# wanxinjin/Learning-from-Sparse-Demonstrations

Hardware: NVIDIA B200
Metric: CPDP OCP gradient-iterations per second (batched quadrotor OCPs, n_grid 50) (higher is better)
Workload: dtype f64

## Files before the change

learning-from-sparse-demonstrations_b200/csrc/cpdp_bdf.cuh:

```cuda
#pragma once
#include "cpdp_aux.cuh"

namespace CPDP_NS {

constexpr int BDF_THREADS = 32;
constexpr int NC = NX + NP;
static_assert(NC <= 32, "k_riccati_bdf maps one lane per column of [P | W]");
static_assert(NX <= 15 && NP <= 16, "warp sections map one lane per row/column and 16 + lane for the second half / the rows of Z; lane 31 must stay free for the bulge-chase fix-up");
#ifndef CPDP_BDF_MINB
#define CPDP_BDF_MINB 8
#endif
constexpr int BDF_MAX_ORDER = 5;
constexpr int BDF_NEWTON_MAXITER = 4;
constexpr int BDF_NROWS = BDF_MAX_ORDER + 3;
constexpr int BDF_WS_DOUBLES = BDF_NROWS * NX * NC;

#ifndef CPDP_BDF_LMUL_UNROLL
#define CPDP_BDF_LMUL_UNROLL 1
#endif
#ifndef CPDP_BDF_STENCIL_UNROLL
#define CPDP_BDF_STENCIL_UNROLL 1
#endif
#ifdef __CUDACC__
#define BDF_SYNC() __syncwarp()
#define BDF_UNROLL _Pragma("unroll")
#define BDF_PRAGMA_STR(x) _Pragma(#x)
#define BDF_PRAGMA_UNROLL(n) BDF_PRAGMA_STR(unroll n)
#else
#define BDF_SYNC() __syncthreads()
#define BDF_UNROLL
#define BDF_PRAGMA_UNROLL(n)
#endif

CPDP_HD double bdf_kappa(int k) { const double v[6] = {0.0, -0.1850, -1.0 / 9, -0.0823, -0.0415, 0.0}; return v[k]; }
CPDP_HD double bdf_gamma(int k) { const double v[6] = {0.0, 1.0, 1.5, 1.8333333333333333, 2.083333333333333, 2.283333333333333}; return v[k]; }
CPDP_HD double bdf_alpha(int k) { return (1.0 - bdf_kappa(k)) * bdf_gamma(k); }
CPDP_HD double bdf_error_const(int k) { return bdf_kappa(k) * bdf_gamma(k) + 1.0 / (k + 1); }

#ifdef __CUDACC__
CPDP_D double bdf_mul(double a, double b) { return __dmul_rn(a, b); }
#else
CPDP_D double bdf_mul(double a, double b) { volatile double r = a * b; return r; }
#endif

constexpr int QS = (NX + 1) & ~1;
constexpr int NCS = NC | 1;
constexpr int SWQ = (NX - 1 + 3) / 4;
constexpr int TW = 4 * SWQ;
constexpr int NH = (NX + 1) / 2;
namespace bo {
constexpr int M = 0;
constexpr int XUL = M + ((MSZ + 1) & ~1);
constexpr int RED = XUL + ((2 * NX + NU + 1) & ~1);
constexpr int Q = RED + 66;
constexpr int QT = Q + NX * QS;
constexpr int WT = QT + NX * QS;
constexpr int LM = WT + NX * QS;
constexpr int Y2 = LM + ((NX * NX + 1) & ~1);
constexpr int T2S = Y2 + 2 * NX * NX;
constexpr int TD = T2S + 2 * NX * TW;
constexpr int PV = TD + 2 * NX;
constexpr int CM = PV + 2 * NX * NX;
constexpr int XA = CM + ((NX * NP + 1) & ~1);
constexpr int XB = XA + NX * NCS;
constexpr int GHM = XB + NX * NCS;
constexpr int YPM = GHM + NX * NU;
constexpr int ROT = YPM + NU * NX;
constexpr int RU = (ROT + 4 * NX + 1) & ~1;
constexpr int FLAG = RU + 128;
constexpr int NODE = FLAG + 2;
constexpr int NODE_W = 2 * NX + NU;
#ifdef CPDP_BDF_TIMING
constexpr int TS = NODE + ((2 * NODE_W + 1) & ~1);
constexpr int END = TS + 8;
#else
constexpr int END = NODE + ((2 * NODE_W + 1) & ~1);
#endif
static_assert(Y2 % 2 == 0 && T2S % 2 == 0 && TD % 2 == 0 && PV % 2 == 0 && RU % 2 == 0, "complex arrays are read with 128-bit loads");
}
constexpr int BDF_SMEM_DOUBLES = bo::END;
constexpr size_t BDF_SMEM_BYTES = (size_t)BDF_SMEM_DOUBLES * sizeof(double);

struct cplx { double x, y; };
#ifdef __CUDACC__
#define BDF_LD2(p) (*reinterpret_cast<const double2*>(p))
#define BDF_ST2(p, a, b) (*reinterpret_cast<double2*>(p) = make_double2((a), (b)))
#else
#define BDF_LD2(p) (*reinterpret_cast<const cplx*>(p))
#define BDF_ST2(p, a, b) do { (p)[0] = (a); (p)[1] = (b); } while (0)
#endif

#define BDF_SM() CPDP_DYN_SMEM(sm)

CPDP_D_NOINLINE double bdf_reduce(double v, bool is_max) {
#ifdef __CUDACC__
    BDF_UNROLL for (int o = 16; o > 0; o >>= 1) {
        const double x = __shfl_xor_sync(0xffffffffu, v, o);
        v = is_max ? fmax(v, x) : (v + x);
    }
    return v;
#else
    BDF_SM();
    return block_reduce(v, sm + bo::RED, is_max);
#endif
}
CPDP_D_NOINLINE double bdf_pow(double x, double y) { return pow(x, y); }
CPDP_D double bdf_rcp(double x) {
#ifdef __CUDACC__
    double r;
    asm("rcp.approx.ftz.f64 %0, %1;" : "=d"(r) : "d"(x));
    r = fma(r, fma(-x, r, 1.0), r);
    r = fma(r, fma(-x, r, 1.0), r);
    return r;
#else
    return 1.0 / x;
#endif
}

#ifdef CPDP_BDF_TIMING
#define BDF_T(ph, ...) do { const long long t0__ = clock64(); __VA_ARGS__; tp[ph] += clock64() - t0__; } while (0)
#define BDF_TB(ph, var, expr) do { const long long t0__ = clock64(); var = (expr); tp[ph] += clock64() - t0__; } while (0)
#define BDF_TP_PARAM , long long* tp
#define BDF_TP_ARG , tp
#define BDF_TS0() const long long ts0__ = clock64()
#define BDF_TS(i) do { if (threadIdx.x == 0) sm[bo::TS + (i)] += (double)(clock64() - ts0__); } while (0)
#else
#define BDF_T(ph, ...) do { __VA_ARGS__; } while (0)
#define BDF_TB(ph, var, expr) do { var = (expr); } while (0)
#define BDF_TP_PARAM
#define BDF_TP_ARG
#define BDF_TS0()
#define BDF_TS(i)
#endif

template <int AS>
CPDP_D_NOINLINE void bdf_lmul_t(const double* __restrict__ AT, const double* __restrict__ x, const int xs,
                                double* __restrict__ dst, const int ds, const int i0) {
    double out[NH];
    BDF_UNROLL for (int i = 0; i < NH; ++i) out[i] = 0.0;
    const double* A0 = AT + i0;
    BDF_PRAGMA_UNROLL(CPDP_BDF_LMUL_UNROLL) for (int k = 0; k < NX; ++k) {
        const double xk = x[k * xs];
        if constexpr (AS % 2 == 0 && (NX - NH) % 2 == 0) {
            double a[NH + 1];
            BDF_UNROLL for (int i = 0; i + 1 < NH + 1; i += 2) { const auto v = BDF_LD2(A0 + k * AS + i); a[i] = v.x; a[i + 1] = v.y; }
            BDF_UNROLL for (int i = 0; i < NH; ++i) out[i] += a[i] * xk;
        } else {
            BDF_UNROLL for (int i = 0; i < NH; ++i) out[i] += A0[k * AS + i] * xk;
        }
    }
    const int first = (i0 > 0) ? 2 * NH - NX : 0;
    BDF_UNROLL for (int i = 0; i < NH; ++i) if (i >= first) dst[(i0 + i) * ds] = out[i];
}
CPDP_D void bdf_lmul_to(const double* AT, const int as, const double* x, const int xs, double* dst, const int ds, const int i0) {
    if (as == QS) bdf_lmul_t<QS>(AT, x, xs, dst, ds, i0);
    else bdf_lmul_t<NCS>(AT, x, xs, dst, ds, i0);
}
CPDP_D bool bdf_half(const int lane, int& col, int& i0) {
    col = lane & 15;
    i0 = (lane >> 4) ? NX - NH : 0;
    return col < NX;
}
CPDP_D void bdf_put(double* buf, int c, const double (&v)[NX]) {
    BDF_UNROLL for (int i = 0; i < NX; ++i) buf[i * NCS + c] = v[i];
}
CPDP_D void bdf_get_col(const double* buf, int c, double (&v)[NX]) {
    BDF_UNROLL for (int i = 0; i < NX; ++i) v[i] = buf[i * NCS + c];
}

CPDP_D void bdf_stage_nodes(double* sm, const AuxProblem& p, const double t0) {
    const int lane = threadIdx.x;
    const int lo = interp_lo(t0, p.dt, p.N);
    BDF_SYNC();
    CPDP_LOOP for (int q = lane; q < 2 * bo::NODE_W; q += BDF_THREADS) {
        const int row = lo + q / bo::NODE_W, e = q % bo::NODE_W;
        sm[bo::NODE + q] = (e < NX) ? p.X[(size_t)row * NX + e]
                         : (e < NX + NU) ? p.U[(size_t)row * NU + e - NX] : p.Lam[(size_t)row * NX + e - NX - NU];
    }
    if (lane == 0) ((int*)(sm + bo::FLAG))[2] = lo;
    BDF_SYNC();
}
CPDP_D_NOINLINE bool bdf_prepare(const AuxProblem p, const double t) {
    BDF_SM();
    const int lane = threadIdx.x;
    BDF_SYNC();
// ... 288 lines not shown
                        pass = (u <= EPS * v);
                    }
                }
                m = bdf_top_bit(bdf_ballot(sm, pass));
                p = bdf_bcast(sm, p, m); q = bdf_bcast(sm, q, m); r = bdf_bcast(sm, r, m);
            }
            BDF_SYNC();
            if (lane == 0 && l >= 1) h_(l, l - 1) = 0.0;
            BDF_TS(1);
            CPDP_LOOP for (int k = m; k <= en - 1; ++k) {
                const bool notlast = (k != en - 1);
                SS(g_ss.steps++);
                if (k != m) { p = h_(k, k - 1); q = h_(k + 1, k - 1); r = notlast ? h_(k + 2, k - 1) : 0.0; }
                const double sig = p * p + q * q + r * r;
                if (sig == 0.0) continue;
                const double rs = bdf_rsqrt(sig);
                const double sgn = (p < 0.0) ? -1.0 : 1.0;
                const double s = sgn * (sig * rs);
                const double xx = 1.0 + fabs(p) * rs, yy = q * rs * sgn, zz = r * rs * sgn;
                const double ixx = bdf_rcp(xx);
                const double qn = yy * ixx, rn = zz * ixx;
                {
                    const bool on = lane >= k && lane < n;
                    double* const col = on ? H + lane : Z;
                    const double a0 = col[k * n], a1 = col[(k + 1) * n], a2 = notlast ? col[(k + 2) * n] : 0.0;
                    const double pp = (a0 + qn * a1) + rn * a2;
                    if (on && notlast) col[(k + 2) * n] = a2 - pp * zz;
                    if (on) col[k * n] = a0 - pp * xx;
                    if (on) col[(k + 1) * n] = a1 - pp * yy;
                }
                BDF_SYNC();
                {
                    const int imax = (en < k + 3) ? en : k + 3;
                    const bool on = lane < 16 ? (rw <= imax) : (rw < n);
                    const double z0 = Mrow[k], z1 = Mrow[k + 1], z2 = notlast ? Mrow[k + 2] : 0.0;
                    const double pp = (xx * z0 + yy * z1) + zz * z2;
                    if (on && notlast) Mrow[k + 2] = z2 - pp * rn;
                    if (on) Mrow[k] = z0 - pp;
                    if (on) Mrow[k + 1] = z1 - pp * qn;
                    if (lane == 31) {
                        if (k != m) { h_(k, k - 1) = -s; h_(k + 1, k - 1) = 0.0; if (notlast) h_(k + 2, k - 1) = 0.0; }
                        else if (l != m) h_(k, k - 1) = -h_(k, k - 1);
                    }
                }
                BDF_SYNC();
            }
            BDF_TS(2);
        }
    }
#undef h_
    return true;
}

CPDP_D_NOINLINE bool bdf_schur() {
    BDF_SM();
    constexpr int n = NX;
    const int lane = threadIdx.x;
    double* Tr = sm + bo::PV; double* Ti = Tr + n * n;
    double* Zm = sm + bo::Y2;
    double* ga = sm + bo::ROT; double* gbr = ga + n; double* gbi = gbr + n; double* pi = gbi + n;
    int* flag = (int*)(sm + bo::FLAG);
    BDF_SYNC();
    CPDP_LOOP for (int e = lane; e < n * n; e += BDF_THREADS) { Tr[e] = sm[bo::LM + e]; Ti[e] = 0.0; }
    if (lane == 0) flag[1] = 1;
    BDF_SYNC();
    const bool ok = schur_real_w0(sm, Tr, Zm, sm + bo::RU);
    BDF_SYNC();
    BDF_TS0();
    if (!ok && lane == 0) flag[1] = 0;
    if (lane < n) { ga[lane] = 1.0; gbr[lane] = 0.0; gbi[lane] = 0.0; pi[lane] = (double)lane; }
    BDF_SYNC();
    CPDP_LOOP for (int j = 0; ok && j < n - 1; ++j) {
        const double cc = Tr[(j + 1) * n + j];
        if (cc == 0.0) continue;
        const double a = Tr[j * n + j], b = Tr[j * n + j + 1], d = Tr[(j + 1) * n + j + 1];
        const double hd = 0.5 * (a - d), disc = hd * hd + b * cc;
        double v1r, v1i;
        if (disc >= 0.0) { v1r = hd + (hd >= 0.0 ? sqrt(disc) : -sqrt(disc)); v1i = 0.0; }
        else { v1r = hd; v1i = sqrt(-disc); }
        const double av1 = sqrt(v1r * v1r + v1i * v1i);
        const double rho = sqrt(av1 * av1 + cc * cc);
        double cr, sr, si;
        if (av1 == 0.0) { cr = 0.0; sr = (cc >= 0.0) ? 1.0 : -1.0; si = 0.0; }
        else { cr = av1 / rho; sr = v1r * cc / (av1 * rho); si = v1i * cc / (av1 * rho); }
        BDF_SYNC();
        if (lane >= j && lane < n) {
            const int k = lane;
            const double xr = Tr[j * n + k], xi = Ti[j * n + k], yr = Tr[(j + 1) * n + k], yi = Ti[(j + 1) * n + k];
            Tr[j * n + k] = cr * xr + (sr * yr - si * yi);
            Ti[j * n + k] = cr * xi + (sr * yi + si * yr);
            Tr[(j + 1) * n + k] = cr * yr - (sr * xr + si * xi);
            Ti[(j + 1) * n + k] = cr * yi - (sr * xi - si * xr);
        }
        BDF_SYNC();
        if (lane <= j + 1) {
            const int k = lane;
            const double xr = Tr[k * n + j], xi = Ti[k * n + j], yr = Tr[k * n + j + 1], yi = Ti[k * n + j + 1];
            Tr[k * n + j] = cr * xr + (sr * yr + si * yi);
            Ti[k * n + j] = cr * xi + (sr * yi - si * yr);
            Tr[k * n + j + 1] = cr * yr - (sr * xr - si * xi);
            Ti[k * n + j + 1] = cr * yi - (sr * xi + si * xr);
        } else if (lane == 16) {
            ga[j] = cr; gbr[j] = sr; gbi[j] = si; pi[j] = (double)(j + 1);
            ga[j + 1] = cr; gbr[j + 1] = -sr; gbi[j + 1] = si; pi[j + 1] = (double)j;
        }
        BDF_SYNC();
        if (lane == 0) { Tr[(j + 1) * n + j] = 0.0; Ti[(j + 1) * n + j] = 0.0; }
        BDF_SYNC();
    }
    BDF_SYNC();
    BDF_TS(3);
    CPDP_LOOP for (int e = lane; e < n * n; e += BDF_THREADS) {
        const int r_ = e / n, c_ = e % n;
        const double v = Zm[e];
        sm[bo::Q + r_ * QS + c_] = v;
        sm[bo::QT + c_ * QS + r_] = v;
    }
    CPDP_LOOP for (int e = lane; e < n * TW; e += BDF_THREADS) {
        const int r_ = e / TW, k = r_ + 1 + e % TW;
        BDF_ST2(sm + bo::T2S + 2 * e, k < n ? Tr[r_ * n + k] : 0.0, k < n ? Ti[r_ * n + k] : 0.0);
    }
    if (lane < n) BDF_ST2(sm + bo::TD + 2 * lane, Tr[lane * n + lane], Ti[lane * n + lane]);
    BDF_SYNC();
    BDF_TS(4);
    return flag[1] != 0;
}

CPDP_D void bdf_stencil_GEGh(const double* rot, const double* E, const int st, const int i, const int j, double& cr, double& ci) {
    constexpr int n = NX;
    const int pi = (int)rot[3 * n + i], pj = (int)rot[3 * n + j];
    const double gi_a = rot[i], gi_br = rot[n + i], gi_bi = rot[2 * n + i];
    const double gj_a = rot[j], gj_br = rot[n + j], gj_bi = -rot[2 * n + j];
    const double c1 = E[i * st + j], c2 = E[pi * st + j], c3 = E[i * st + pj], c4 = E[pi * st + pj];
    const double ujr = gi_a * c1 + gi_br * c2, uji = gi_bi * c2;
    const double upr = gi_a * c3 + gi_br * c4, upi = gi_bi * c4;
    cr = ujr * gj_a + (upr * gj_br - upi * gj_bi);
    ci = uji * gj_a + (upr * gj_bi + upi * gj_br);
}
CPDP_D double bdf_stencil_GhYG(const double* rot, const double* Y, const int i, const int j) {
    constexpr int n = NX;
    const int pi = (int)rot[3 * n + i], pj = (int)rot[3 * n + j];
    const double ai_r = rot[i], ap_r = rot[n + pi], ap_i = -rot[2 * n + pi];
    const double bj_r = rot[j], bp_r = rot[n + pj], bp_i = rot[2 * n + pj];
    const bool hi = (pi != i), hj = (pj != j);
    const auto y1 = BDF_LD2(Y + 2 * (i * n + j)), y2 = BDF_LD2(Y + 2 * (pi * n + j));
    const auto y3 = BDF_LD2(Y + 2 * (i * n + pj)), y4 = BDF_LD2(Y + 2 * (pi * n + pj));
    const double tjr = ai_r * y1.x + (hi ? (ap_r * y2.x - ap_i * y2.y) : 0.0);
    const double tpr = ai_r * y3.x + (hi ? (ap_r * y4.x - ap_i * y4.y) : 0.0), tpi = ai_r * y3.y + (hi ? (ap_r * y4.y + ap_i * y4.x) : 0.0);
    return tjr * bj_r + (hj ? (tpr * bp_r - tpi * bp_i) : 0.0);
}

CPDP_D_NOINLINE bool bdf_factor(const double c) {
    BDF_SM();
    constexpr int n = NX;
    const int lane = threadIdx.x;
    const bool isP = lane < n, isB = (lane >= 16) && (lane < 16 + n);
    const double* TD = sm + bo::TD;
    double* XA = sm + bo::XA; double* XB = sm + bo::XB;
    BDF_SYNC();
    double bad = 0.0;
    if (isP) {
        const int j = lane;
        const auto tj = BDF_LD2(TD + 2 * j);
        CPDP_LOOP for (int i = 0; i <= j; ++i) {
            const auto ti = BDF_LD2(TD + 2 * i);
            const double er = 1.0 + c * (ti.x + tj.x), ei = c * (ti.y - tj.y);
            const double ee = er * er + ei * ei;
            if (!(ee > 0.0)) bad = 1.0;
            const double ie = 1.0 / ee;
            BDF_ST2(sm + bo::PV + 2 * (i * n + j), er * ie, -ei * ie);
        }
        BDF_UNROLL for (int i = 0; i < n; ++i) XA[i * NCS + j] = ((i == j) ? 1.0 : 0.0) + c * sm[bo::LM + i * n + j];
    } else if (isB) {
        BDF_UNROLL for (int i = 0; i < n; ++i) XB[i * NCS + lane - 16] = (i == lane - 16) ? 1.0 : 0.0;
    }
    double* mine = isP ? XA + lane : XB + (isB ? lane - 16 : 0);
    const bool own = isP || isB;
    BDF_SYNC();
    CPDP_LOOP for (int k = 0; k < n; ++k) {
        const int p = bdf_argmax(sm, (isP && lane >= k) ? XA[lane * NCS + k] : 0.0, isP && lane >= k);
        if (p < 0) { bad = 1.0; break; }
        if (own && p != k) { const double a = mine[k * NCS], b = mine[p * NCS]; mine[k * NCS] = b; mine[p * NCS] = a; }
        BDF_SYNC();
        double ak[n];
        BDF_UNROLL for (int i = 0; i < n; ++i) ak[i] = XA[i * NCS + k];
        const double ip = bdf_rcp(XA[k * NCS + k]);
        BDF_SYNC();
        if (own) {
            const double t = mine[k * NCS] * ip;
            BDF_UNROLL for (int i = 0; i < n; ++i) mine[i * NCS] -= ak[i] * t;
            mine[k * NCS] = t;
        }
        BDF_SYNC();
    }
    if (bdf_ballot(sm, bad != 0.0)) return false;
    if (isB) { BDF_UNROLL for (int i = 0; i < n; ++i) sm[bo::WT + (lane - 16) * QS + i] = XB[i * NCS + lane - 16]; }
    BDF_SYNC();
    return true;
}

CPDP_D void bdf_sweep(double* sm, const double c) {
    constexpr int n = NX;
    const int tid = threadIdx.x;
    const double* T2 = sm + bo::T2S; double* Y = sm + bo::Y2; const double* PVm = sm + bo::PV;
    const int e = tid >> 2, sub = tid & 3;
    static_assert(bo::Y2 - 2 * 7 * NX >= 0 && bo::T2S - 2 * 8 * TW >= 0, "sweep: idle-lane operands below the arrays");
    static_assert(bo::Y2 + 2 * ((NX + 7 + 4 * SWQ) * NX + NX) <= bo::END && bo::T2S + 2 * ((NX + 7) * TW + 4 * SWQ) <= bo::END,
                  "sweep: idle-lane operands beyond the arrays");
    int d = 2 * (n - 1);
    int i = (n - 1) + e, j = d - i;
#ifdef __CUDACC__
// ... 30 lines not shown
        }
        const auto cv = BDF_LD2(cvp), pv = BDF_LD2(pvp);
        BDF_UNROLL for (int w = 1; w < 2 * SWQ; w *= 2) {
            BDF_UNROLL for (int m = 0; m + w < 2 * SWQ; m += 2 * w) { pr[m] += pr[m + w]; pi_[m] += pi_[m + w]; }
        }
        double ar = pr[0], ai = pi_[0];
#ifdef __CUDACC__
        ar += __shfl_xor_sync(0xffffffffu, ar, 1); ai += __shfl_xor_sync(0xffffffffu, ai, 1);
        ar += __shfl_xor_sync(0xffffffffu, ar, 2); ai += __shfl_xor_sync(0xffffffffu, ai, 2);
#else
        double* red = sm + bo::RED;
        __syncthreads();
        red[tid] = ar; red[32 + tid] = ai;
        __syncthreads();
        if (sub == 0) {
            ar = (red[tid] + red[tid + 1]) + (red[tid + 2] + red[tid + 3]);
            ai = (red[32 + tid] + red[32 + tid + 1]) + (red[32 + tid + 2] + red[32 + tid + 3]);
        }
#endif
        {
            const double rr = cv.x - c * ar, ri = cv.y - c * ai;
            const double yr = rr * pv.x - ri * pv.y, yi = rr * pv.y + ri * pv.x;
            const bool st = valid && (sub == 0);
            double* dump = sm + bo::RU + 2 * tid;
#ifdef __CUDACC__
            double* p1 = st ? Y + oij : dump;
            double* p2 = (st && i != j) ? Y + oji : dump + 64;
#else
            double* p1 = st ? Y + 2 * (i * n + j) : dump;
            double* p2 = (st && i != j) ? Y + 2 * (j * n + i) : dump + 64;
#endif
            BDF_ST2(p1, yr, (i == j) ? 0.0 : yi);
            BDF_ST2(p2, yr, -yi);
        }
        const bool up = d > n - 1;
        if (up) --i; else --j;
#ifdef __CUDACC__
        oti -= up ? 2 * TW : 0; otj -= up ? 0 : 2 * TW;
        oij -= up ? 2 * n : 2; oji -= up ? 2 : 2 * n;
#endif
        BDF_SYNC();
    }
}

CPDP_D void bdf_solve_cols(double* sm, const double c, double (&r)[NX] BDF_TP_PARAM) {
    constexpr int n = NX;
    const int lane = threadIdx.x;
    const bool isP = lane < n, isW = (lane >= n) && (lane < NC);
    const int j = isP ? lane : 0;
    const double* rot = sm + bo::ROT;
    double* XA = sm + bo::XA; double* XB = sm + bo::XB;
    int hc, hi0;
    const bool hact = bdf_half(lane, hc, hi0);
    BDF_T(10, {
    if (isP) bdf_put(XA, j, r);
    BDF_SYNC();
    if (hact) bdf_lmul_to(sm + bo::Q, QS, XA + hc, NCS, XB + hc, NCS, hi0);
    BDF_SYNC();
    if (hact) bdf_lmul_to(sm + bo::Q, QS, XB + hc * NCS, 1, XA + hc, NCS, hi0);
    BDF_SYNC();
    });
    BDF_T(11, {
    if (isP) {
        BDF_PRAGMA_UNROLL(CPDP_BDF_STENCIL_UNROLL) for (int i = 0; i <= j; ++i) {
            double cr, ci;
            bdf_stencil_GEGh(rot, XA, NCS, i, j, cr, ci);
            BDF_ST2(sm + bo::Y2 + 2 * (i * n + j), cr, ci);
        }
    }
    BDF_SYNC();
    });
    BDF_T(12, { bdf_sweep(sm, c); BDF_SYNC(); });
    BDF_T(13, {
    if (isP) {
        BDF_PRAGMA_UNROLL(CPDP_BDF_STENCIL_UNROLL) for (int i = 0; i < n; ++i) XA[i * NCS + j] = bdf_stencil_GhYG(rot, sm + bo::Y2, i, j);
    }
    BDF_SYNC();
    });
    BDF_T(14, {
    if (hact) bdf_lmul_to(sm + bo::QT, QS, XA + hc, NCS, XB + hc, NCS, hi0);
    BDF_SYNC();
    if (hact) bdf_lmul_to(sm + bo::QT, QS, XB + hc * NCS, 1, XA + hc, NCS, hi0);
    BDF_SYNC();
    });
    BDF_T(15, {
    double xs_[NX];
    if (isP) { BDF_UNROLL for (int i = 0; i < n; ++i) xs_[i] = 0.5 * (XA[i * NCS + j] + XA[j * NCS + i]); }
    BDF_SYNC();
    if (isP) {
        BDF_UNROLL for (int i = 0; i < n; ++i) r[i] = xs_[i];
        bdf_put(XA, j, r);
    }
    BDF_SYNC();
    const int wc = lane & 15, wi0 = (lane >> 4) ? NX - NH : 0;
    if (wc < NP) bdf_lmul_to(XA, NCS, sm + bo::CM + wc, NP, XB + n + wc, NCS, wi0);
    BDF_SYNC();
    if (isW) { BDF_UNROLL for (int i = 0; i < n; ++i) XB[i * NCS + lane] = r[i] + c * XB[i * NCS + lane]; }
    BDF_SYNC();
    if (wc < NP) bdf_lmul_to(sm + bo::WT, QS, XB + n + wc, NCS, XA + n + wc, NCS, wi0);
    BDF_SYNC();
    if (isW) { BDF_UNROLL for (int i = 0; i < n; ++i) r[i] = XA[i * NCS + lane]; }
    BDF_SYNC();
    });
}

CPDP_D_NOINLINE void bdf_change_D(double* D, const int order, const double factor) {
    BDF_SM();
    const int lane = threadIdx.x;
    double* RU = sm + bo::RU; double* R = RU + 36; double* U = RU + 72;
    BDF_SYNC();
    if (lane <= order) {
        const int j = lane;
        R[j] = 1.0; U[j] = 1.0;
        CPDP_LOOP for (int i = 1; i <= order; ++i) {
            R[i * 6 + j] = (j == 0) ? 0.0 : R[(i - 1) * 6 + j] * (((double)(i - 1) - factor * j) / i);
            U[i * 6 + j] = (j == 0) ? 0.0 : U[(i - 1) * 6 + j] * (((double)(i - 1) - (double)j) / i);
        }
    }
    BDF_SYNC();
    CPDP_LOOP for (int e = lane; e < 36; e += BDF_THREADS) {
        const int i = e / 6, j = e % 6;
        if (i <= order && j <= order) {
            double acc = 0.0;
            CPDP_LOOP for (int k = 0; k <= order; ++k) acc += R[i * 6 + k] * U[k * 6 + j];
            RU[i * 6 + j] = acc;
        }
    }
    BDF_SYNC();
    if (lane < NC) {
        CPDP_LOOP for (int q = 0; q < NX; ++q) {
            double* Dq = D + (size_t)q * NC + lane;
            double v[BDF_MAX_ORDER + 1];
            BDF_UNROLL for (int i = 0; i <= BDF_MAX_ORDER; ++i) v[i] = (i <= order) ? Dq[(size_t)i * NX * NC] : 0.0;
// ... 2 lines not shown
                    double acc = 0.0;
                    BDF_UNROLL for (int jj = 0; jj <= BDF_MAX_ORDER; ++jj) if (jj <= order) acc += RU[jj * 6 + i] * v[jj];
                    Dq[(size_t)i * NX * NC] = acc;
                }
            }
        }
    }
    BDF_SYNC();
}

CPDP_D double bdf_norm_cols(const double (&v)[NX], const double (&isc)[NX], const double mul, const bool act) {
    double a = 0.0;
    if (act) { BDF_UNROLL for (int i = 0; i < NX; ++i) { const double x = mul * v[i] * isc[i]; a += x * x; } }
    return sqrt(bdf_reduce(a, false) / (double)NFULL_R);
}
CPDP_D_NOINLINE double bdf_norm_row(const double* Drow, const double* iscm, const double mul) {
    const int lane = threadIdx.x;
    double a = 0.0;
    if (lane < NC) { BDF_UNROLL for (int i = 0; i < NX; ++i) { const double x = mul * Drow[(size_t)i * NC + lane] * iscm[i * NCS + lane]; a += x * x; } }
    return sqrt(bdf_reduce(a, false) / (double)NFULL_R);
}

CPDP_D_NOINLINE void bdf_rhs_smem(const bool sym) {
    BDF_SM();
    const int c = threadIdx.x < NC ? threadIdx.x : 0;
    double y[NX], f[NX];
    bdf_get_col(sm + bo::XB, c, y);
    BDF_SYNC();
    bdf_rhs_cols(sm, y, f, sym);
    if (threadIdx.x < NC) bdf_put(sm + bo::XB, c, f);
    BDF_SYNC();
}

CPDP_D int bdf_interval(double* sm, double* D, const AuxProblem& p, const double t0, const double t1,
                        const double rtol, const double atol, double (&y)[NX], int* cnt BDF_TP_PARAM) {
    const int lane = threadIdx.x;
    const bool act = lane < NC;
    const int lc = act ? lane : 0;
    const double dir = (t1 >= t0) ? 1.0 : -1.0;
    const double EPS = 2.220446049250313e-16;
#define D_(row, i) D[((size_t)(row) * NX + (i)) * NC + lc]
    bdf_stage_nodes(sm, p, t0);
    { bool okp__; BDF_TB(0, okp__, bdf_prepare(p, t0)); if (!okp__) return 2; }
    double f0[NX];
    if (act) bdf_put(sm + bo::XA, lc, y);
    BDF_SYNC();
    BDF_T(2, bdf_jacobian()); ++cnt[3];
    if (act) bdf_put(sm + bo::XB, lc, y);
    BDF_SYNC();
    BDF_T(1, bdf_rhs_smem(true)); ++cnt[0];
    bdf_get_col(sm + bo::XB, lc, f0);
    BDF_SYNC();
    { bool oks__; BDF_TB(3, oks__, bdf_schur()); if (!oks__) return 4; }
    double h_abs;
    {
        const double interval_length = fabs(t1 - t0);
        double a0 = 0.0, a1 = 0.0;
        double isc0[NX];
        BDF_UNROLL for (int i = 0; i < NX; ++i) isc0[i] = bdf_rcp(atol + fabs(y[i]) * rtol);
        if (act) {
            BDF_UNROLL for (int i = 0; i < NX; ++i) {
                a0 += (y[i] * isc0[i]) * (y[i] * isc0[i]);
                a1 += (f0[i] * isc0[i]) * (f0[i] * isc0[i]);
            }
        }
        const double d0 = sqrt(bdf_reduce(a0, false) / (double)NFULL_R);
        const double d1 = sqrt(bdf_reduce(a1, false) / (double)NFULL_R);
        double h0 = (d0 < 1e-5 || d1 < 1e-5) ? 1e-6 : 0.01 * d0 / d1;
        h0 = fmin(h0, interval_length);
        double f1[NX];
        if (act) { BDF_UNROLL for (int i = 0; i < NX; ++i) f1[i] = y[i] + h0 * dir * f0[i]; bdf_put(sm + bo::XB, lc, f1); }
        { bool okp__; BDF_TB(0, okp__, bdf_prepare(p, t0 + h0 * dir)); if (!okp__) return 2; }
        BDF_T(1, bdf_rhs_smem(true)); ++cnt[0];
        bdf_get_col(sm + bo::XB, lc, f1);
        BDF_SYNC();
        double a2 = 0.0;
        if (act) {
            BDF_UNROLL for (int i = 0; i < NX; ++i) {
                const double v = (f1[i] - f0[i]) * isc0[i];
                a2 += v * v;
            }
        }
        const double d2 = sqrt(bdf_reduce(a2, false) / (double)NFULL_R) / h0;
        double h1;
        if (d1 <= 1e-15 && d2 <= 1e-15) h1 = fmax(1e-6, h0 * 1e-3);
        else h1 = bdf_pow(0.01 / fmax(d1, d2), 1.0 / 2.0);
        h_abs = fmin(fmin(100 * h0, h1), interval_length);
    }
    const double newton_tol = fmax(10 * EPS / rtol, fmin(0.03, sqrt(rtol)));
    if (act) { BDF_UNROLL for (int i = 0; i < NX; ++i) { D_(0, i) = y[i]; D_(1, i) = f0[i] * h_abs * dir; } }
    BDF_SYNC();
    int order = 1, n_equal_steps = 0;
    bool lu_valid = false;
    double c_lu = 0.0;
    double t = t0;
    double d[NX], psi[NX], isc[NX];
    BDF_UNROLL for (int i = 0; i < NX; ++i) { d[i] = 0.0; psi[i] = 0.0; isc[i] = 0.0; }

    while (dir * (t - t1) < 0) {
        const double min_step = 10 * fabs(nextafter(t, dir * INFINITY) - t);
        if (h_abs < min_step) {
            BDF_T(7, bdf_change_D(D, order, min_step / h_abs));
            h_abs = min_step;
            n_equal_steps = 0;
        }
        bool current_jac = false;
        double t_new = t, error_norm = 0.0, safety = 0.0;
        int n_iter = 0;
        while (true) {
            if (h_abs < min_step) return 1;
            double h = h_abs * dir;
            t_new = t + h;
            if (dir * (t_new - t1) > 0) {
                t_new = t1;
                BDF_T(7, bdf_change_D(D, order, fabs(t_new - t) / h_abs));
                n_equal_steps = 0;
                lu_valid = false;
            }
            h = t_new - t;
            h_abs = fabs(h);
            const double al = bdf_alpha(order), ial = 1.0 / al;
            if (act) {
                double dk[NX];
                BDF_UNROLL for (int i = 0; i < NX; ++i) { y[i] = 0.0; psi[i] = 0.0; }
                CPDP_LOOP for (int k = 0; k <= order; ++k) {
                    const double gk = bdf_gamma(k);
                    BDF_UNROLL for (int i = 0; i < NX; ++i) dk[i] = D_(k, i);
                    BDF_UNROLL for (int i = 0; i < NX; ++i) { y[i] += dk[i]; psi[i] += dk[i] * gk; }
                }
                BDF_UNROLL for (int i = 0; i < NX; ++i) {
                    isc[i] = bdf_rcp(atol + rtol * fabs(y[i]));
                    psi[i] = psi[i] * ial;
                }
            }
            { bool okp__; BDF_TB(0, okp__, bdf_prepare(p, t_new)); if (!okp__) return 2; }
            const double c = h / al;
            bool converged = false;
            while (!converged) {
                if (!lu_valid) {
                    { bool okf__; BDF_TB(4, okf__, bdf_factor(c)); if (!okf__) return 4; }
                    lu_valid = true; c_lu = c; ++cnt[2];
                }
                BDF_UNROLL for (int i = 0; i < NX; ++i) d[i] = 0.0;
                double dy_norm_old = -1.0;
                int k = 0;
                CPDP_LOOP for (k = 0; k < BDF_NEWTON_MAXITER; ++k) {
                    double r[NX];
                    if (act) bdf_put(sm + bo::XB, lc, y);
                    BDF_SYNC();
                    BDF_T(1, bdf_rhs_smem(false)); ++cnt[0];
                    bdf_get_col(sm + bo::XB, lc, r);
                    bool fin = false;
                    BDF_UNROLL for (int i = 0; i < NX; ++i) {
                        if (act && !(fabs(r[i]) < 1e300)) fin = true;
                        r[i] = c * r[i] - psi[i] - d[i];
                    }
                    if (bdf_ballot(sm, fin)) break;
                    BDF_T(5, bdf_solve_cols(sm, c_lu, r BDF_TP_ARG));
                    double dy_norm; BDF_TB(6, dy_norm, bdf_norm_cols(r, isc, 1.0, act));
                    const bool have_rate = dy_norm_old >= 0.0;
                    const double rate = have_rate ? dy_norm / dy_norm_old : 0.0;
                    double rpow = rate;
                    if (BDF_NEWTON_MAXITER - k >= 2) rpow *= rate;
                    if (BDF_NEWTON_MAXITER - k >= 3) rpow *= rate;
                    static_assert(BDF_NEWTON_MAXITER == 4, "rate power above is written for exponents <= 3");
                    if (have_rate && (rate >= 1 || rpow / (1 - rate) * dy_norm > newton_tol)) break;
                    BDF_UNROLL for (int i = 0; i < NX; ++i) { y[i] += r[i]; d[i] += r[i]; }
                    if (dy_norm == 0 || (have_rate && rate / (1 - rate) * dy_norm < newton_tol)) { converged = true; break; }
                    dy_norm_old = dy_norm;
                }
                n_iter = (k < BDF_NEWTON_MAXITER) ? k + 1 : BDF_NEWTON_MAXITER;
                if (!converged) {
                    if (current_jac) break;
                    if (act) {
                        BDF_UNROLL for (int i = 0; i < NX; ++i) y[i] = 0.0;
                        CPDP_LOOP for (int kk = 0; kk <= order; ++kk) { BDF_UNROLL for (int i = 0; i < NX; ++i) y[i] += D_(kk, i); }
                        bdf_put(sm + bo::XA, lc, y);
                    }
                    BDF_SYNC();
                    BDF_T(2, bdf_jacobian()); ++cnt[3];
                    { bool oks__; BDF_TB(3, oks__, bdf_schur()); if (!oks__) return 4; }
                    lu_valid = false;
                    current_jac = true;
                }
            }
            if (!converged) {
                h_abs *= 0.5;
                BDF_T(7, bdf_change_D(D, order, 0.5));
                n_equal_steps = 0;
                lu_valid = false;
                continue;
            }
            safety = 0.9 * (2 * BDF_NEWTON_MAXITER + 1) / (double)(2 * BDF_NEWTON_MAXITER + n_iter);
            BDF_UNROLL for (int i = 0; i < NX; ++i) isc[i] = bdf_rcp(atol + rtol * fabs(y[i]));
            BDF_TB(6, error_norm, bdf_norm_cols(d, isc, bdf_error_const(order), act));
            if (!(error_norm == error_norm)) return 2;
            if (error_norm > 1) {
                const double factor = fmax(0.2, safety * bdf_pow(error_norm, -1.0 / (order + 1)));
                h_abs *= factor;
                BDF_T(7, bdf_change_D(D, order, factor));
                n_equal_steps = 0;
            } else {
                break;
            }
        }
        ++n_equal_steps;
        ++cnt[1];
        t = t_new;
        const bool sel_order = !(n_equal_steps < order + 1);
        if (act) {
            double up[NX];
            BDF_UNROLL for (int i = 0; i < NX; ++i) up[i] = D_(order + 1, i);
            BDF_UNROLL for (int i = 0; i < NX; ++i) { D_(order + 2, i) = d[i] - up[i]; D_(order + 1, i) = d[i]; up[i] = d[i]; }
            CPDP_LOOP for (int k = order; k >= 0; --k) {
                double cur[NX];
                BDF_UNROLL for (int i = 0; i < NX; ++i) cur[i] = D_(k, i);
                BDF_UNROLL for (int i = 0; i < NX; ++i) { up[i] += cur[i]; D_(k, i) = up[i]; }
            }
            if (sel_order) { BDF_UNROLL for (int i = 0; i < NX; ++i) sm[bo::XB + i * NCS + lc] = isc[i]; }
        }
        BDF_SYNC();
        if (!sel_order) continue;
        double error_m_norm = INFINITY, error_p_norm = INFINITY;
        if (order > 1) BDF_TB(6, error_m_norm, bdf_norm_row(D + (size_t)order * NX * NC, sm + bo::XB, bdf_error_const(order - 1)));
        if (order < BDF_MAX_ORDER) BDF_TB(6, error_p_norm, bdf_norm_row(D + (size_t)(order + 2) * NX * NC, sm + bo::XB, bdf_error_const(order + 1)));
        const double fm = bdf_pow(error_m_norm, -1.0 / order);
        const double f0_ = bdf_pow(error_norm, -1.0 / (order + 1));
        const double fp = bdf_pow(error_p_norm, -1.0 / (order + 2));
        int delta_order = -1; double fmaxv = fm;
        if (f0_ > fmaxv) { fmaxv = f0_; delta_order = 0; }
        if (fp > fmaxv) { fmaxv = fp; delta_order = 1; }
        order += delta_order;
        const double factor = fmin(10.0, safety * fmaxv);
        h_abs *= factor;
        BDF_T(7, bdf_change_D(D, order, factor));
        n_equal_steps = 0;
        lu_valid = false;
    }
    if (act) { BDF_UNROLL for (int i = 0; i < NX; ++i) y[i] = D_(0, i); }
    BDF_SYNC();
#undef D_
    return 0;
}

CPDP_GLOBAL void __launch_bounds__(BDF_THREADS, CPDP_BDF_MINB) k_riccati_bdf(AuxArgs a) {
    const int b = blockIdx.x, lane = threadIdx.x;
    if (a.solve_status && (a.solve_status[b] == ST_NUMERIC || a.solve_status[b] == ST_RUNNING)) {
        if (lane == 0) a.aux_status[b] = 3;
        return;
    }
    BDF_SM();
    const bool act = lane < NC, isP = lane < NX;
    const int lc = act ? lane : 0;
    CPDP_LOOP for (int q = lane; q < MSZ; q += BDF_THREADS) sm[bo::M + q] = 0.0;
    double* D = a.Dws + (size_t)b * BDF_WS_DOUBLES;
    const int N = a.N;
    AuxProblem p;
    p.X = a.X + (size_t)b * (N + 1) * NX; p.U = a.U + (size_t)b * (N + 1) * NU; p.Lam = a.Lam + (size_t)b * (N + 1) * NX;
    p.th = a.theta + (size_t)b * a.theta_stride; p.pd = a.pdata + (size_t)b * NQ; p.PW = nullptr; p.dt = a.T / N; p.N = N;
    double* PW = a.PW + (size_t)b * (N + 1) * NYR;
    double* s_hxx = sm + bo::PV; double* s_hxe = sm + bo::XA;
    if (lane == 0) {
        const double tN = p.dt * N;
        double xT[NX];
        const int lo = interp_lo(tN, p.dt, N);
        CPDP_LOOP for (int i = 0; i < NX; ++i) xT[i] = interp_val(p.X[(size_t)lo * NX + i], p.X[(size_t)(lo + 1) * NX + i], p.dt * lo, p.dt * (lo + 1), tN);
        PdBuf pdb;
        Model::term2(xT, p.th, pd_at(p.pd, tN, pdb), s_hxx, s_hxe);
    }
    BDF_SYNC();
    double y[NX];
    BDF_UNROLL for (int i = 0; i < NX; ++i) {
        y[i] = isP ? 0.5 * (s_hxx[i * NX + lc] + s_hxx[lc * NX + i]) : s_hxe[i * NP + (act ? lc - NX : 0)];
    }
    BDF_SYNC();
#define BDF_STORE_NODE(k_)                                                                              \
    if (act) {                                                                                          \
        BDF_UNROLL for (int i = 0; i < NX; ++i) {                                                       \
            if (isP) { if (i <= lc) PW[(size_t)(k_) * NYR + tri(i, lc)] = y[i]; }                       \
            else PW[(size_t)(k_) * NYR + NT + i * NP + (lc - NX)] = y[i];                               \
        }                                                                                               \
    }
    BDF_STORE_NODE(N)
    int cnt[4] = {0, 0, 0, 0};
    int st = 0;
#ifdef CPDP_BDF_TIMING
    long long tp[16] = {0, 0, 0, 0, 0, 0, 0, 0, 0, 0, 0, 0, 0, 0, 0, 0};
    if (lane < 8) sm[bo::TS + lane] = 0.0;
    const long long tstart__ = clock64();
#endif
    CPDP_LOOP for (int k = N; k >= 1 && st == 0; --k) {
        st = bdf_interval(sm, D, p, p.dt * k, p.dt * (k - 1), a.rtol_b, a.atol_b, y, cnt BDF_TP_ARG);
        BDF_STORE_NODE(k - 1)
        BDF_SYNC();
    }
#undef BDF_STORE_NODE
#ifdef CPDP_BDF_TIMING
    if (lane == 0) {
        tp[8] = clock64() - tstart__;
        double* dst = a.Ua + (size_t)b * (N + 1) * NU * NP;
        for (int i = 0; i < 16; ++i) dst[i] = (double)tp[i];
        for (int i = 0; i < 8; ++i) dst[16 + i] = sm[bo::TS + i];
    }
#endif
    if (lane == 0) {
        a.aux_status[b] = st;
        a.counters[b * NCOUNTERS + 0] = cnt[0]; a.counters[b * NCOUNTERS + 1] = cnt[1];
        a.counters[b * NCOUNTERS + 4] = cnt[2]; a.counters[b * NCOUNTERS + 5] = cnt[3];
    }
}


constexpr int RKW_K_DOUBLES = 7 * NX * NC;
constexpr bool RKW_K_OVERLAID = RKW_K_DOUBLES <= bo::XA - bo::Q;
constexpr int RKW_K = RKW_K_OVERLAID ? bo::Q : ((bo::END + 1) & ~1);
constexpr int RKW_SMEM_DOUBLES = RKW_K_OVERLAID ? bo::END : RKW_K + RKW_K_DOUBLES;
constexpr size_t RKW_SMEM_BYTES = (size_t)RKW_SMEM_DOUBLES * sizeof(double);

CPDP_D bool rkw_rhs(double* sm, const AuxProblem& p, const double t, const bool with_prepare, const double (&yin)[NX], const int stage,
                    const bool act, const int lc) {
    if (with_prepare && !bdf_prepare(p, t)) return false;
    if (act) bdf_put(sm + bo::XB, lc, yin);
    BDF_SYNC();
    bdf_rhs_smem(true);
    if (act) { BDF_UNROLL for (int i = 0; i < NX; ++i) sm[RKW_K + (stage * NX + i) * NC + lc] = sm[bo::XB + i * NCS + lc]; }
    BDF_SYNC();
    return true;
}

CPDP_D int rkw_interval(double* sm, const AuxProblem& p, const double t0, const double t1, const double rtol, const double atol,
                        double (&y)[NX], int& nrhs, int& nsteps) {
    const int lane = threadIdx.x;
    const bool act = lane < NC;
    const int lc = act ? lane : 0;
    const double dir = (t1 >= t0) ? 1.0 : -1.0;
    const double NF = (double)NFULL_R;
#define K_(s_, i_) sm[RKW_K + ((s_) * NX + (i_)) * NC + lc]
    bdf_stage_nodes(sm, p, t0);
    if (!rkw_rhs(sm, p, t0, true, y, 0, act, lc)) return 2;
    ++nrhs;
    double h_abs;
    {
        const double interval_length = fabs(t1 - t0);
        double a0 = 0.0, a1 = 0.0;
        if (act) {
            BDF_UNROLL for (int i = 0; i < NX; ++i) {
                const double sc = atol + fabs(y[i]) * rtol;
                const double f = K_(0, i);
                a0 += (y[i] / sc) * (y[i] / sc);
                a1 += (f / sc) * (f / sc);
            }
        }
        const double d0 = sqrt(bdf_reduce(a0, false) / NF);
        const double d1 = sqrt(bdf_reduce(a1, false) / NF);
        double h0 = (d0 < 1e-5 || d1 < 1e-5) ? 1e-6 : 0.01 * d0 / d1;
        h0 = fmin(h0, interval_length);
// ... 128 lines not shown
```

Measured before the change: 27120.

## Diagonalize the BDF Jacobian via an eigenbasis instead of the Schur-based Sylvester solve

After the real Schur decomposition, the code now computes eigenvectors of the quasi-triangular factor and their inverse. When the eigenbasis condition estimate is below a threshold, it uses a diagonal (elementwise) Lyapunov/Sylvester factorization and solve in place of the complex Givens reduction and triangular stencil back-substitution. This is meant to replace the per-Newton-iteration sequential triangular solve with a parallel elementwise scaling between basis changes. The cost is an extra eigenvector and inverse computation at each Jacobian refactorization, plus some loss of accuracy for ill-conditioned bases, which is why the condition guard falls back to the old path.

```diff
diff --git a/learning-from-sparse-demonstrations_b200/csrc/cpdp_bdf.cuh b/learning-from-sparse-demonstrations_b200/csrc/cpdp_bdf.cuh
--- a/learning-from-sparse-demonstrations_b200/csrc/cpdp_bdf.cuh
+++ b/learning-from-sparse-demonstrations_b200/csrc/cpdp_bdf.cuh
@@ -21,6 +21,10 @@
 #ifndef CPDP_BDF_STENCIL_UNROLL
 #define CPDP_BDF_STENCIL_UNROLL 1
 #endif
+#ifndef CPDP_BDF_EIG_KAPPA
+#define CPDP_BDF_EIG_KAPPA 1e4
+#endif
+constexpr double BDF_EIG_KAPPA = CPDP_BDF_EIG_KAPPA;
 #ifdef __CUDACC__
 #define BDF_SYNC() __syncwarp()
 #define BDF_UNROLL _Pragma("unroll")
@@ -77,6 +81,7 @@
 constexpr int END = NODE + ((2 * NODE_W + 1) & ~1);
 #endif
 static_assert(Y2 % 2 == 0 && T2S % 2 == 0 && TD % 2 == 0 && PV % 2 == 0 && RU % 2 == 0, "complex arrays are read with 128-bit loads");
+static_assert(2 * NX * NX <= T2S - Y2 && NX * NX <= 2 * NX * TW && NX * QS <= 2 * NX * TW, "eigen path scratch");
 }
 constexpr int BDF_SMEM_DOUBLES = bo::END;
 constexpr size_t BDF_SMEM_BYTES = (size_t)BDF_SMEM_DOUBLES * sizeof(double);
@@ -131,6 +136,14 @@
 #define BDF_TP_ARG
 #define BDF_TS0()
 #define BDF_TS(i)
+#endif
+#ifdef CPDP_BDF_TIMING
+#define CPDP_BDF_PATH_COUNTS
+#endif
+#ifdef CPDP_BDF_PATH_COUNTS
+#define BDF_PATH(sm, k) do { cnt[4 + (k) + ((BDF_EIG_KAPPA > 0.0 && ((const int*)((sm) + bo::FLAG))[3]) ? 0 : 1)] += 1; } while (0)
+#else
+#define BDF_PATH(sm, k) do { } while (0)
 #endif
 
 template <int AS>
@@ -525,6 +538,109 @@
     return true;
 }
 
+CPDP_D bool bdf_eig_basis(double* sm, const double* T) {
+    constexpr int n = NX;
+    const int lane = threadIdx.x;
+    const bool own = lane < n;
+    const int j = own ? lane : 0;
+    double* Vr = sm + bo::Y2; double* Vi = Vr + n * n; double* W = sm + bo::T2S;
+    const bool up = j + 1 < n && T[(j + 1) * n + j] != 0.0, dn = j >= 1 && T[j * n + j - 1] != 0.0;
+    const int bs = dn ? j - 1 : j, be = up ? j + 1 : j;
+    double lr = T[j * n + j], li = 0.0;
+    double x0r = 1.0, x0i = 0.0, x1r = 0.0;
+    bool cpx = false;
+    if (bs != be) {
+        const double p = T[bs * n + bs], q = T[bs * n + be], r = T[be * n + bs], s = T[be * n + be];
+        const double hd = 0.5 * (p - s), disc = hd * hd + q * r;
+        if (disc < 0.0) { cpx = true; li = sqrt(-disc); lr = s + hd; x0r = hd; x0i = li; x1r = r; }
+        else {
+            const double sq = (hd >= 0.0) ? sqrt(disc) : -sqrt(disc);
+            if (j == bs) { lr = s + (hd + sq); x0r = hd + sq; x1r = r; }
+            else { lr = p - (hd + sq); x0r = q; x1r = -(hd + sq); }
+        }
+    }
+    if (own) {
+        CPDP_LOOP for (int i = 0; i < n; ++i) { Vr[i * n + j] = 0.0; Vi[i * n + j] = 0.0; }
+        Vr[bs * n + j] = x0r; Vi[bs * n + j] = x0i;
+        if (be != bs) Vr[be * n + j] = x1r;
+    }
+    for (int i = n - 1; i >= 0;) {
+        const bool two = i >= 1 && T[i * n + i - 1] != 0.0;
+        const int i0 = two ? i - 1 : i;
+        if (own && i < bs) {
+            double ar = 0.0, ai = 0.0, br = 0.0, bi = 0.0;
+            CPDP_LOOP for (int m = i + 1; m < n; ++m) {
+                const double xr = Vr[m * n + j], xi = Vi[m * n + j], ta = T[i0 * n + m], tb = T[i * n + m];
+                ar -= ta * xr; ai -= ta * xi; br -= tb * xr; bi -= tb * xi;
+            }
+            const double dr = T[i0 * n + i0] - lr, di = -li;
+            double yr, yi;
+            if (two) {
+                const double er = T[i * n + i] - lr, t01 = T[i0 * n + i], t10 = T[i * n + i0];
+                const double gr = (dr * er - di * di) - t01 * t10, gi = dr * di + di * er;
+                const double ig = 1.0 / (gr * gr + gi * gi);
+                const double ur = (ar * er - ai * di) - t01 * br, ui = (ar * di + ai * er) - t01 * bi;
+                const double wr = (dr * br - di * bi) - t10 * ar, wi = (dr * bi + di * br) - t10 * ai;
+                Vr[i0 * n + j] = (ur * gr + ui * gi) * ig; Vi[i0 * n + j] = (ui * gr - ur * gi) * ig;
+                yr = (wr * gr + wi * gi) * ig; yi = (wi * gr - wr * gi) * ig;
+            } else {
+                const double ig = 1.0 / (dr * dr + di * di);
+                yr = (ar * dr + ai * di) * ig; yi = (ai * dr - ar * di) * ig;
+            }
+            Vr[i * n + j] = yr; Vi[i * n + j] = yi;
+        }
+        i = i0 - 1;
+    }
+    if (own) {
+        double s2 = 0.0;
+        CPDP_LOOP for (int m = 0; m < n; ++m) s2 += Vr[m * n + j] * Vr[m * n + j] + Vi[m * n + j] * Vi[m * n + j];
+        const double sc = 1.0 / sqrt(s2);
+        const double* src = (cpx && j == be) ? Vi : Vr;
+        CPDP_LOOP for (int m = 0; m < n; ++m) Vr[m * n + j] = src[m * n + j] * sc;
+    }
+    BDF_SYNC();
+    for (int i = n - 1; i >= 0;) {
+        const bool two = i >= 1 && T[i * n + i - 1] != 0.0;
+        const int i0 = two ? i - 1 : i;
+        if (own) {
+            double a = (i0 == j) ? 1.0 : 0.0, b = (i == j) ? 1.0 : 0.0;
+            CPDP_LOOP for (int m = i + 1; m < n; ++m) { const double w = W[m * n + j]; a -= Vr[i0 * n + m] * w; b -= Vr[i * n + m] * w; }
+            if (two) {
+                const double v00 = Vr[i0 * n + i0], v01 = Vr[i0 * n + i], v10 = Vr[i * n + i0], v11 = Vr[i * n + i];
+                const double ig = 1.0 / (v00 * v11 - v01 * v10);
+                W[i0 * n + j] = (a * v11 - v01 * b) * ig;
+                W[i * n + j] = (v00 * b - v10 * a) * ig;
+            } else {
+                W[i * n + j] = a / Vr[i * n + i];
+            }
+        }
+        i = i0 - 1;
+    }
+    double nv = 0.0, nw = 0.0;
+    if (own) { CPDP_LOOP for (int m = 0; m < n; ++m) { nv += Vr[m * n + j] * Vr[m * n + j]; nw += W[m * n + j] * W[m * n + j]; } }
+    nv = bdf_reduce(nv, false);
+    nw = bdf_reduce(nw, false);
+    if (!(nv * nw <= BDF_EIG_KAPPA * BDF_EIG_KAPPA)) return false;
+    double* XA = sm + bo::XA; double* XB = sm + bo::XB;
+    int hc, hi0;
+    if (bdf_half(lane, hc, hi0)) {
+        bdf_lmul_to(sm + bo::QT, QS, Vr + hc, n, XA + hc, NCS, hi0);
+        bdf_lmul_to(sm + bo::QT, QS, W + hc * n, 1, XB + hc, NCS, hi0);
+    }
+    BDF_SYNC();
+    CPDP_LOOP for (int e = lane; e < n * n; e += BDF_THREADS) {
+        const int k = e / n, i = e % n;
+        sm[bo::Q + k * QS + i] = XB[k * NCS + i];
+        sm[bo::QT + k * QS + i] = XA[i * NCS + k];
+    }
+    if (own) {
+        BDF_ST2(sm + bo::TD + 2 * j, lr, li);
+        sm[bo::ROT + 3 * n + j] = (double)(cpx ? (j == bs ? be : bs) : j);
+    }
+    BDF_SYNC();
+    return true;
+}
+
 CPDP_D_NOINLINE bool bdf_schur() {
     BDF_SM();
     constexpr int n = NX;
@@ -539,8 +655,23 @@
     BDF_SYNC();
     const bool ok = schur_real_w0(sm, Tr, Zm, sm + bo::RU);
     BDF_SYNC();
+    if (!ok && lane == 0) flag[1] = 0;
+    CPDP_LOOP for (int e = lane; e < n * n; e += BDF_THREADS) {
+        const int r_ = e / n, c_ = e % n;
+        const double v = Zm[e];
+        sm[bo::Q + r_ * QS + c_] = v;
+        sm[bo::QT + c_ * QS + r_] = v;
+    }
+    BDF_SYNC();
+    if (BDF_EIG_KAPPA > 0.0) {
+        BDF_TS0();
+        const bool eig = ok && bdf_eig_basis(sm, Tr);
+        if (lane == 0) flag[3] = eig ? 1 : 0;
+        BDF_SYNC();
+        BDF_TS(5);
+        if (eig) return true;
+    }
     BDF_TS0();
-    if (!ok && lane == 0) flag[1] = 0;
     if (lane < n) { ga[lane] = 1.0; gbr[lane] = 0.0; gbi[lane] = 0.0; pi[lane] = (double)lane; }
     BDF_SYNC();
     CPDP_LOOP for (int j = 0; ok && j < n - 1; ++j) {
@@ -583,12 +714,6 @@
     }
     BDF_SYNC();
     BDF_TS(3);
-    CPDP_LOOP for (int e = lane; e < n * n; e += BDF_THREADS) {
-        const int r_ = e / n, c_ = e % n;
-        const double v = Zm[e];
-        sm[bo::Q + r_ * QS + c_] = v;
-        sm[bo::QT + c_ * QS + r_] = v;
-    }
     CPDP_LOOP for (int e = lane; e < n * TW; e += BDF_THREADS) {
         const int r_ = e / TW, k = r_ + 1 + e % TW;
         BDF_ST2(sm + bo::T2S + 2 * e, k < n ? Tr[r_ * n + k] : 0.0, k < n ? Ti[r_ * n + k] : 0.0);
@@ -623,6 +748,47 @@
     return tjr * bj_r + (hj ? (tpr * bp_r - tpi * bp_i) : 0.0);
 }
 
+CPDP_D bool bdf_factor_eig(double* sm, const double c) {
+    constexpr int n = NX;
+    const int lane = threadIdx.x;
+    const bool own = lane < n;
+    const int j = own ? lane : 0;
+    const double* TD = sm + bo::TD; const double* part = sm + bo::ROT + 3 * n;
+    double* s1 = sm + bo::ROT; double* s2 = s1 + n;
+    double* XA = sm + bo::XA;
+    BDF_SYNC();
+    double bad = 0.0;
+    if (own) {
+        const auto lj = BDF_LD2(TD + 2 * j);
+        const int pj = (int)part[j];
+        const double sj = (pj > j) ? 1.0 : ((pj < j) ? -1.0 : 0.0);
+        CPDP_LOOP for (int i = 0; i < n; ++i) {
+            const auto li = BDF_LD2(TD + 2 * i);
+            const int pi = (int)part[i];
+            const double si = (pi > i) ? 1.0 : ((pi < i) ? -1.0 : 0.0);
+            const double er = 1.0 + c * (li.x + lj.x), ep = c * (li.y - lj.y), em = -c * (li.y + lj.y);
+            const double mp = er * er + ep * ep, mm = er * er + em * em;
+            if (!(mp > 0.0) || !(mm > 0.0)) bad = 1.0;
+            const double ip = 1.0 / mp, im = 1.0 / mm;
+            const double u = er * ip, v = -ep * ip, w = er * im, t = -em * im;
+            BDF_ST2(sm + bo::PV + 2 * (i * n + j), 0.5 * (u + w), si * (0.5 * (v - t)));
+            BDF_ST2(sm + bo::Y2 + 2 * (i * n + j), -sj * (0.5 * (v + t)), (si * sj) * (0.5 * (u - w)));
+        }
+        const double dr = 1.0 + c * lj.x, di = c * lj.y, md = dr * dr + di * di;
+        if (!(md > 0.0)) bad = 1.0;
+        s1[j] = dr / md; s2[j] = sj * (-di / md);
+    }
+    BDF_SYNC();
+    if (own) {
+        CPDP_LOOP for (int i = 0; i < n; ++i) XA[i * NCS + j] = s1[i] * sm[bo::Q + j * QS + i] + s2[i] * sm[bo::Q + j * QS + (int)part[i]];
+    }
+    BDF_SYNC();
+    int hc, hi0;
+    if (bdf_half(lane, hc, hi0)) bdf_lmul_to(sm + bo::QT, QS, XA + hc, NCS, sm + bo::WT + hc * QS, 1, hi0);
+    BDF_SYNC();
+    return !bdf_ballot(sm, bad != 0.0);
+}
+
 CPDP_D_NOINLINE bool bdf_factor(const double c) {
     BDF_SM();
     constexpr int n = NX;
@@ -630,6 +796,7 @@
     const bool isP = lane < n, isB = (lane >= 16) && (lane < 16 + n);
     const double* TD = sm + bo::TD;
     double* XA = sm + bo::XA; double* XB = sm + bo::XB;
+    if (BDF_EIG_KAPPA > 0.0 && ((const int*)(sm + bo::FLAG))[3]) return bdf_factor_eig(sm, c);
     BDF_SYNC();
     double bad = 0.0;
     if (isP) {
@@ -766,6 +933,8 @@
     double* XA = sm + bo::XA; double* XB = sm + bo::XB;
     int hc, hi0;
     const bool hact = bdf_half(lane, hc, hi0);
+    const bool eig = BDF_EIG_KAPPA > 0.0 && ((const int*)(sm + bo::FLAG))[3];
+    double* ZB = sm + bo::T2S;
     BDF_T(10, {
     if (isP) bdf_put(XA, j, r);
     BDF_SYNC();
@@ -774,6 +943,20 @@
     if (hact) bdf_lmul_to(sm + bo::Q, QS, XB + hc * NCS, 1, XA + hc, NCS, hi0);
     BDF_SYNC();
     });
+    if (eig) {
+    BDF_T(9, {
+    if (isP) {
+        const double* part = rot + 3 * n;
+        const int pj = (int)part[j];
+        CPDP_LOOP for (int i = 0; i < n; ++i) {
+            const int pi = (int)part[i];
+            const auto k12 = BDF_LD2(sm + bo::PV + 2 * (i * n + j)), k34 = BDF_LD2(sm + bo::Y2 + 2 * (i * n + j));
+            ZB[i * QS + j] = ((k12.x * XA[i * NCS + j] + k12.y * XA[pi * NCS + j]) + k34.x * XA[i * NCS + pj]) + k34.y * XA[pi * NCS + pj];
+        }
+    }
+    BDF_SYNC();
+    });
+    } else {
     BDF_T(11, {
     if (isP) {
         BDF_PRAGMA_UNROLL(CPDP_BDF_STENCIL_UNROLL) for (int i = 0; i <= j; ++i) {
@@ -791,8 +974,9 @@
     }
     BDF_SYNC();
     });
+    }
     BDF_T(14, {
-    if (hact) bdf_lmul_to(sm + bo::QT, QS, XA + hc, NCS, XB + hc, NCS, hi0);
+    if (hact) bdf_lmul_to(sm + bo::QT, QS, (eig ? ZB : XA) + hc, eig ? QS : NCS, XB + hc, NCS, hi0);
     BDF_SYNC();
     if (hact) bdf_lmul_to(sm + bo::QT, QS, XB + hc * NCS, 1, XA + hc, NCS, hi0);
     BDF_SYNC();
@@ -901,6 +1085,7 @@
     bdf_get_col(sm + bo::XB, lc, f0);
     BDF_SYNC();
     { bool oks__; BDF_TB(3, oks__, bdf_schur()); if (!oks__) return 4; }
+    BDF_PATH(sm, 2);
     double h_abs;
     {
         const double interval_length = fabs(t1 - t0);
@@ -1006,6 +1191,7 @@
                     }
                     if (bdf_ballot(sm, fin)) break;
                     BDF_T(5, bdf_solve_cols(sm, c_lu, r BDF_TP_ARG));
+                    BDF_PATH(sm, 0);
                     double dy_norm; BDF_TB(6, dy_norm, bdf_norm_cols(r, isc, 1.0, act));
                     const bool have_rate = dy_norm_old >= 0.0;
                     const double rate = have_rate ? dy_norm / dy_norm_old : 0.0;
@@ -1029,6 +1215,7 @@
                     BDF_SYNC();
                     BDF_T(2, bdf_jacobian()); ++cnt[3];
                     { bool oks__; BDF_TB(3, oks__, bdf_schur()); if (!oks__) return 4; }
+                    BDF_PATH(sm, 2);
                     lu_valid = false;
                     current_jac = true;
                 }
@@ -1131,7 +1318,7 @@
         }                                                                                               \
     }
     BDF_STORE_NODE(N)
-    int cnt[4] = {0, 0, 0, 0};
+    int cnt[8] = {0, 0, 0, 0, 0, 0, 0, 0};
     int st = 0;
 #ifdef CPDP_BDF_TIMING
     long long tp[16] = {0, 0, 0, 0, 0, 0, 0, 0, 0, 0, 0, 0, 0, 0, 0, 0};
@@ -1151,6 +1338,9 @@
         for (int i = 0; i < 16; ++i) dst[i] = (double)tp[i];
         for (int i = 0; i < 8; ++i) dst[16 + i] = sm[bo::TS + i];
     }
+#endif
+#ifdef CPDP_BDF_PATH_COUNTS
+    if (lane == 0) { for (int i = 0; i < 4; ++i) a.Ua[(size_t)b * (N + 1) * NU * NP + 24 + i] = (double)cnt[4 + i]; }
 #endif
     if (lane == 0) {
         a.aux_status[b] = st;
```

New measurement: 29970 (median of 6 runs). 10.5% higher.
